# lucidrains/phenaki-pytorch

Hardware: AMD Instinct MI355X
Metric: cvivit_encode_frames_per_sec (higher is better)
Workload: dtype bf16; 1 GPU; BASELINE configs[1]: C-ViViT (dim 512, patch 32, tpatch 2, depth 4+4, LFQ 65536) encode video -> token ids, (8,3,17,256,256) f32 per GPU resident in HBM; global_batch=8, parallelism=batch-shard x1, no data-path collective, hip_graph=True

## Files before the change

phenaki_pytorch_amd/csrc/gemm.hip:

```cpp
#include "gemm_dma.hpp"
#include "gemm_p8.hpp"

namespace pk {

enum { ACT_NONE = 0, ACT_GEGLU = 1, ACT_LEAKY = 2 };

struct GemmEpilogue {
    const float* bias;
    const float* res;
    void* C;
    int ldr, ldc;
    int out_f32;
    int act;
    int vec_ok;
    void* C2;
    int ldc2;
    const float* ln_s; const float* ln_t; float ln_eps;
    const int* row_off; const int* col_off;
    float* stats_out; const float* ln_stats; int stats_np;
    int dup_rows;
};

constexpr int STATS_CHUNK = 32;

// ... 151 lines not shown
    gemm_epilogue<T, TM, TN>(acc, p.M, p.N, e, m0, n0);
}

template <typename Tile>
constexpr int lds_waves_per_simd() {
    const int wgs = 163840 / Tile::SMEM, w = wgs * (Tile::THREADS / 64) / 4;
    return w < 1 ? 1 : (w > 8 ? 8 : w);
}

template <typename T, int TM, int TN, int WM, int WN, int STAGES, int ROWB, int PW, int LNF = 0>
__global__ __launch_bounds__(64 * (WM * WN + PW))
__attribute__((amdgpu_waves_per_eu(lds_waves_per_simd<GemmDma<T, TM, TN, WM, WN, STAGES, ROWB, PW>>(), 8)))
void gemm_dma_kernel(const GemmOperands p, const GemmEpilogue e, int a_nrows) {
    using Tile = GemmDma<T, TM, TN, WM, WN, STAGES, ROWB, PW>;
    extern __shared__ __attribute__((aligned(16))) char smem[];
    const int MT = (p.M + Tile::BM - 1) / Tile::BM, cmax = (MT + 7) / 8, NTn = (p.N + Tile::BN - 1) / Tile::BN;
    const int xcd = blockIdx.x & 7, idx = blockIdx.x >> 3;
    const int mstart = xcd * MT / 8, mcount = (xcd + 1) * MT / 8 - mstart;
    int m0, n0;
    if (p.plain_map) {
        if ((int)blockIdx.x >= MT * NTn) return;
        m0 = (blockIdx.x % MT) * Tile::BM;
        n0 = (blockIdx.x / MT) * Tile::BN;
    } else {
        int ml, ntile;
        if (!xcd_panel_tile(idx, cmax, mcount, NTn, p.panel, ml, ntile)) return;
        m0 = (mstart + ml) * Tile::BM;
        n0 = ntile * Tile::BN;
    }
    PK_TL_KERNEL(0);
    f32x4 acc[TM][TN];
#pragma unroll
    for (int i = 0; i < TM; ++i)
#pragma unroll
        for (int j = 0; j < TN; ++j) acc[i][j] = f32x4{0, 0, 0, 0};
    if constexpr (LNF == 1) {
        float rsum[TM], rsq[TM];
        if (!Tile::template run_stats<2>(p, a_nrows, m0, n0, smem, acc, rsum, rsq)) return;
        gemm_epilogue<T, TM, TN, WN, true>(acc, p.M, p.N, e, m0, n0, rsum, rsq, p.K);
    } else if constexpr (LNF == 2) {
        constexpr int TPR = Tile::THREADS / Tile::BM;
        static_assert(Tile::THREADS == TPR * Tile::BM && (TPR == 2 || TPR == 4), "2 or 4 threads per tile row");
        constexpr int NPRE = 16 / TPR;
        const int srow = threadIdx.x / TPR, sq4 = threadIdx.x % TPR;
        const int per = (e.stats_np + TPR - 1) / TPR, c0 = sq4 * per, c1 = min(c0 + per, e.stats_np);
        const float2* st = reinterpret_cast<const float2*>(e.ln_stats) + (size_t)min(m0 + srow, p.M - 1) * e.stats_np;
        float su = 0.f, sq = 0.f;
        for (int c = c0 + NPRE; c < c1; ++c) { const float2 pr = st[c]; su += pr.x; sq += pr.y; }
        float2 pre[NPRE];
#pragma unroll
        for (int u = 0; u < NPRE; ++u) pre[u] = c0 + u < c1 ? st[c0 + u] : float2{0.f, 0.f};
        if (!Tile::run(p, a_nrows, m0, n0, smem, acc)) return;
#pragma unroll
        for (int u = 0; u < NPRE; ++u) { su += pre[u].x; sq += pre[u].y; }
        su += __shfl_xor(su, 1); sq += __shfl_xor(sq, 1);
        if (TPR == 4) { su += __shfl_xor(su, 2); sq += __shfl_xor(sq, 2); }
        __syncthreads();
        float2* ls = reinterpret_cast<float2*>(smem);
        if (sq4 == 0) ls[srow] = float2{su, sq};
        __syncthreads();
        float rsum[TM], rsq[TM];
        const int lane = threadIdx.x & 63, wm = (threadIdx.x >> 6) / WN;
#pragma unroll
        for (int i = 0; i < TM; ++i) { const float2 pr = ls[wm * 16 * TM + i * 16 + (lane & 15)]; rsum[i] = pr.x; rsq[i] = pr.y; }
        gemm_epilogue<T, TM, TN, WN, true>(acc, p.M, p.N, e, m0, n0, rsum, rsq, p.K);
    } else {
        if (!Tile::run(p, a_nrows, m0, n0, smem, acc)) return;
        PK_TL_KERNEL(1);
        gemm_epilogue<T, TM, TN, WN>(acc, p.M, p.N, e, m0, n0);
        asm volatile("s_waitcnt vmcnt(0)" ::: "memory");
        PK_TL_KERNEL(2);
    }
}

template <typename T, int TM, int TN, int WM, int WN, int STAGES>
__global__ __launch_bounds__(64 * WM * WN)
__attribute__((amdgpu_waves_per_eu(lds_waves_per_simd<GemmDma<T, TM, TN, WM, WN, STAGES, 128, 0>>(), 8)))
void gemm_dma_splitk_kernel(GemmOperands p, GemmEpilogue e, int a_nrows, long batch_a, long batch_w, long batch_c) {
    using Tile = GemmDma<T, TM, TN, WM, WN, STAGES, 128, 0>;
    extern __shared__ __attribute__((aligned(16))) char smem[];
    const int z = blockIdx.y;
    p.A = reinterpret_cast<const char*>(p.A) + (size_t)z * batch_a;
    p.W = reinterpret_cast<const char*>(p.W) + (size_t)z * batch_w;
    e.C = reinterpret_cast<char*>(e.C) + (size_t)z * batch_c;
    if (z != 0) e.bias = nullptr;
    const int MT = (p.M + Tile::BM - 1) / Tile::BM, NTn = (p.N + Tile::BN - 1) / Tile::BN;
// ... 26 lines not shown
    PK_CHECK_LAUNCH();
    return PK_OK;
}

template <typename T, int TM, int TN, int STAGES, int WM = 2, int WN = 2, int ROWB = 128, int PW = 0, int LNF = 0>
static int launch_dma(const GemmOperands& p, const GemmEpilogue& e, int a_nrows, hipStream_t s) {
    using Tile = GemmDma<T, TM, TN, WM, WN, STAGES, ROWB, PW>;
    if (Tile::SMEM > 65536) {
        static LdsOptIn lds;
        if (lds.raise(reinterpret_cast<const void*>(&gemm_dma_kernel<T, TM, TN, WM, WN, STAGES, ROWB, PW, LNF>), Tile::SMEM) != PK_OK) return PK_ELAUNCH;
    }
    const int MT = (p.M + Tile::BM - 1) / Tile::BM, NT = (p.N + Tile::BN - 1) / Tile::BN;
    dim3 grid(8 * ((MT + 7) / 8) * NT);
    GemmOperands pp = p;
    static const int panel_env = [] { const char* e_ = getenv("PK_GEMM_PANEL"); return e_ ? atoi(e_) : -1; }();
    pp.panel = panel_env >= 0 ? panel_env : xcd_panel_rows(Tile::BM, p.K, (int)sizeof(T));
    hipLaunchKernelGGL((gemm_dma_kernel<T, TM, TN, WM, WN, STAGES, ROWB, PW, LNF>), grid, dim3(Tile::THREADS), Tile::SMEM, s, pp, e, a_nrows);
    PK_CHECK_LAUNCH();
    return PK_OK;
}

__global__ __launch_bounds__(512) __attribute__((amdgpu_waves_per_eu(2, 2)))
void gemm_p8_kernel(const GemmOperands p, const GemmEpilogue e, int a_nrows) {
    using Tile = GemmP8;
    extern __shared__ __attribute__((aligned(16))) char smem[];
    const int MT = (p.M + Tile::BM - 1) / Tile::BM, cmax = (MT + 7) / 8, NTn = (p.N + Tile::BN - 1) / Tile::BN;
    const int xcd = blockIdx.x & 7, idx = blockIdx.x >> 3;
    const int mstart = xcd * MT / 8, mcount = (xcd + 1) * MT / 8 - mstart;
    int m0, n0;
    if (p.plain_map) {
        if ((int)blockIdx.x >= MT * NTn) return;
        m0 = (blockIdx.x % MT) * Tile::BM;
        n0 = (blockIdx.x / MT) * Tile::BN;
    } else {
        int ml, ntile;
        if (!xcd_panel_tile(idx, cmax, mcount, NTn, p.panel, ml, ntile)) return;
        m0 = (mstart + ml) * Tile::BM;
        n0 = ntile * Tile::BN;
    }
    Tile::Acc acc;
#pragma unroll
    for (int a = 0; a < 2; ++a)
#pragma unroll
        for (int b = 0; b < 2; ++b)
#pragma unroll
            for (int i = 0; i < 4; ++i)
#pragma unroll
                for (int j = 0; j < 2; ++j) acc[a][b][i][j] = f32x4{0, 0, 0, 0};
    Tile::run(p, a_nrows, m0, n0, smem, acc);
    gemm_epilogue<bf16, 4, 2, 4>(acc[0][0], p.M, p.N, e, m0, n0);
    gemm_epilogue<bf16, 4, 2, 4>(acc[0][1], p.M, p.N, e, m0, n0 + 128);
    gemm_epilogue<bf16, 4, 2, 4>(acc[1][0], p.M, p.N, e, m0 + 128, n0);
    gemm_epilogue<bf16, 4, 2, 4>(acc[1][1], p.M, p.N, e, m0 + 128, n0 + 128);
}

static int launch_p8(const GemmOperands& p, const GemmEpilogue& e, int a_nrows, hipStream_t s) {
    using Tile = GemmP8;
    static LdsOptIn lds;
    if (lds.raise(reinterpret_cast<const void*>(&gemm_p8_kernel), Tile::SMEM) != PK_OK) return PK_ELAUNCH;
    const int MT = (p.M + Tile::BM - 1) / Tile::BM, NT = (p.N + Tile::BN - 1) / Tile::BN;
    dim3 grid(8 * ((MT + 7) / 8) * NT);
    GemmOperands pp = p;
    static const int panel_env = [] { const char* e_ = getenv("PK_GEMM_PANEL"); return e_ ? atoi(e_) : -1; }();
    pp.panel = panel_env >= 0 ? panel_env : xcd_panel_rows(Tile::BM, p.K, (int)sizeof(bf16));
    hipLaunchKernelGGL(gemm_p8_kernel, grid, dim3(Tile::THREADS), Tile::SMEM, s, pp, e, a_nrows);
    PK_CHECK_LAUNCH();
    return PK_OK;
}

__global__ __launch_bounds__(512) __attribute__((amdgpu_waves_per_eu(2, 2)))
void gemm_p8_splitk_kernel(GemmOperands p, GemmEpilogue e, int a_nrows, long batch_a, long batch_w, long batch_c) {
    using Tile = GemmP8;
    extern __shared__ __attribute__((aligned(16))) char smem[];
    const int z = blockIdx.y;
    p.A = reinterpret_cast<const char*>(p.A) + (size_t)z * batch_a;
    p.W = reinterpret_cast<const char*>(p.W) + (size_t)z * batch_w;
    e.C = reinterpret_cast<char*>(e.C) + (size_t)z * batch_c;
    if (z != 0) e.bias = nullptr;
    const int MT = (p.M + Tile::BM - 1) / Tile::BM, NTn = (p.N + Tile::BN - 1) / Tile::BN;
// ... 80 lines not shown
    e.vec_ok = v ? 1 : 0;
    if (C2 && (!v || !out_is_f32 || act == ACT_GEGLU || dtype != 1 || (ldc2 & 3) || (reinterpret_cast<uintptr_t>(C2) & 7))) return PK_EINVAL;
    if ((ln_s == nullptr) != (ln_t == nullptr)) return PK_EINVAL;
    if ((row_off == nullptr) != (col_off == nullptr)) return PK_EINVAL;
    if (row_off && (!v || !out_is_f32 || act == ACT_GEGLU || res || C2)) return PK_EINVAL;
    if (ln_stats && (!ln_s || stats_out || (reinterpret_cast<uintptr_t>(ln_stats) & 7))) return PK_EINVAL;
    if (stats_out && (!v || act == ACT_GEGLU || row_off || (reinterpret_cast<uintptr_t>(stats_out) & 7))) return PK_EINVAL;
    if (dup_rows < 0 || (dup_rows && (!v || act == ACT_GEGLU || row_off || stats_out || dup_rows < M))) return PK_EINVAL;
    hipStream_t s = reinterpret_cast<hipStream_t>(stream);

    const bool dma_ok = dma_possible(dtype, a_is_f32, N, K, lda, ldw, a_nrows);
    if (variant >= 100) { p.plain_map = 1; variant -= 100; }
    if (variant == 0) variant = auto_variant(dtype, a_is_f32, M, N, K, lda, ldw, a_nrows);
    if (variant >= 3 && !dma_ok) return PK_EINVAL;
    if (ln_s) {
        if (!dma_ok || !v || !al16(ln_s) || !al16(ln_t) || a_rows) return PK_EINVAL;
        const bool big = variant == 24 || variant == 2 || variant == 9 || variant == 50;
        if (ln_stats) {
            if (dtype == 1) return big ? launch_dma<bf16, 4, 2, 2, 2, 4, 128, 0, 2>(p, e, a_nrows, s) : launch_dma<bf16, 2, 2, 2, 2, 2, 128, 0, 2>(p, e, a_nrows, s);
            if (dtype == 2) return big ? launch_dma<bf16x3, 4, 4, 2, 2, 2, 128, 0, 2>(p, e, a_nrows, s) : launch_dma<bf16x3, 2, 2, 2, 2, 2, 128, 0, 2>(p, e, a_nrows, s);
            return big ? launch_dma<float, 4, 2, 2, 2, 4, 128, 0, 2>(p, e, a_nrows, s) : launch_dma<float, 2, 2, 2, 2, 2, 128, 0, 2>(p, e, a_nrows, s);
        }
        if (dtype == 1) return big ? launch_dma<bf16, 4, 2, 2, 2, 4, 128, 0, 1>(p, e, a_nrows, s) : launch_dma<bf16, 2, 2, 2, 2, 2, 128, 0, 1>(p, e, a_nrows, s);
        if (dtype == 2) return big ? launch_dma<bf16x3, 4, 4, 2, 2, 2, 128, 0, 1>(p, e, a_nrows, s) : launch_dma<bf16x3, 2, 2, 2, 2, 2, 128, 0, 1>(p, e, a_nrows, s);
        return big ? launch_dma<float, 4, 2, 2, 2, 4, 128, 0, 1>(p, e, a_nrows, s) : launch_dma<float, 2, 2, 2, 2, 2, 128, 0, 1>(p, e, a_nrows, s);
    }
    if (stats_out && !(dma_ok && (variant == 8 || variant == 24 || variant == 27 || variant == 33 || variant == 50 || (variant == 3 && dtype != 1)))) return PK_EINVAL;
    if (dtype == 1) {
        switch (variant) {
            case 1: return a_is_f32 ? launch_v1<bf16, float, 2, 2>(p, e, s) : launch_v1<bf16, bf16, 2, 2>(p, e, s);
            case 2: return a_is_f32 ? launch_v1<bf16, float, 4, 4>(p, e, s) : launch_v1<bf16, bf16, 4, 4>(p, e, s);
// ... 78 lines not shown
```

phenaki_pytorch_amd/csrc/gemm_core.hpp:

```cpp
#pragma once
#include <cstdlib>
#include "common.hpp"

namespace pk {

static inline int krot_default() {
    static const int v = getenv("PK_GEMM_KROT") ? atoi(getenv("PK_GEMM_KROT")) : 1;
    return v;
}

struct GemmOperands {
    const void* A;
    const void* W;
    const int* a_rows;
    int lda, ldw;
    int M, N, K;
    int plain_map;
    int krot;
    int w_gap_from, w_gap_rows;
    int panel;
};

__device__ __forceinline__ bool xcd_panel_tile(int idx, int cmax, int mcount, int NT, int panel, int& ml, int& ntile) {
    if (panel <= 0 || panel >= cmax) { ml = idx % cmax; ntile = idx / cmax; }
    else {
        const int full = cmax / panel;
        int pi = idx / (panel * NT);
        if (pi > full) pi = full;
        const int base = pi * panel;
        const int pl = pi < full ? panel : cmax - base;
        const int r = idx - pi * panel * NT;
        ml = base + r % pl;
        ntile = r / pl;
    }
    return ml < mcount;
}
static inline int xcd_panel_rows(int BM, int K, int esz) {
    const long tile_bytes = (long)BM * K * esz;
    long pnl = (1 << 20) / (tile_bytes > 0 ? tile_bytes : 1);
    return (int)(pnl < 4 ? 4 : pnl);
}

template <typename T, typename TA> struct RawSlot;
template <typename T> struct RawSlot<T, T> { u32x4 v; };
template <> struct RawSlot<bf16, float> { f32x4 a, b; };

template <typename T>
__device__ __forceinline__ void raw_load(RawSlot<T, T>& r, const T* p, bool ok) {
    r.v = ok ? *reinterpret_cast<const u32x4*>(p) : u32x4{0, 0, 0, 0};
// ... 124 lines not shown
```

phenaki_pytorch_amd/csrc/gemm_dma.hpp:

```cpp
#pragma once
#include "gemm_core.hpp"

namespace pk {

__device__ __forceinline__ void dot2acc_bf16(float& d, uint32_t a, uint32_t b) {
    asm("v_dot2c_f32_bf16 %0, %1, %2" : "+v"(d) : "v"(a), "v"(b));
}
__device__ __forceinline__ void frag_stats(const Frag<bf16>& f, float& s, float& q, bool want_sq) {
    const uint32_t w0 = f.v[0], w1 = f.v[1], w2 = f.v[2], w3 = f.v[3];
    const uint32_t ones = 0x3f803f80u;
    dot2acc_bf16(s, w0, ones); dot2acc_bf16(s, w1, ones); dot2acc_bf16(s, w2, ones); dot2acc_bf16(s, w3, ones);
    if (want_sq) { dot2acc_bf16(q, w0, w0); dot2acc_bf16(q, w1, w1); dot2acc_bf16(q, w2, w2); dot2acc_bf16(q, w3, w3); }
}
__device__ __forceinline__ void frag_stats(const Frag<float>& f, float& s, float& q, bool want_sq) {
#pragma unroll
    for (int e = 0; e < 4; ++e) {
        s += f.lo[e] + f.hi[e];
        if (want_sq) q = fmaf(f.lo[e], f.lo[e], fmaf(f.hi[e], f.hi[e], q));
    }
}

#ifdef PK_TIMELINE
__device__ unsigned long long pk_tl[8 * 5 * 40];
#define PK_TL(slot) do { if (tl_on && kt < 38) pk_tl[(tl_wg * 40 + kt) * 5 + (slot)] = __builtin_amdgcn_s_memtime(); } while (0)
// ... 40 lines not shown

    template <int TILES> static __device__ __forceinline__ void wait_tiles() { wait_vmcnt<TILES * IPW>(); }

    static __device__ __forceinline__ void wait_outstanding(int tiles) {
        switch (tiles) {
            case 0: wait_tiles<0>(); break;
            case 1: wait_tiles<1>(); break;
            case 2: wait_tiles<(STAGES > 3 ? 2 : 0)>(); break;
            case 3: wait_tiles<(STAGES > 4 ? 3 : 0)>(); break;
            case 4: wait_tiles<(STAGES > 5 ? 4 : 0)>(); break;
            case 5: wait_tiles<(STAGES > 6 ? 5 : 0)>(); break;
            default: wait_tiles<(STAGES > 7 ? 6 : 0)>(); break;
        }
    }

    static __device__ __forceinline__ bool run(const GemmOperands& p, int a_nrows, int m0, int n0, char* smem, f32x4 (&acc)[TM][TN]) {
        float dummy[TM];
        return run_stats<0>(p, a_nrows, m0, n0, smem, acc, dummy, dummy);
    }

    template <int STATS>
    static __device__ __forceinline__ bool run_stats(const GemmOperands& p, int a_nrows, int m0, int n0, char* smem, f32x4 (&acc)[TM][TN],
                                                     float (&rsum)[TM], float (&rsq)[TM]) {
        const int tid = threadIdx.x, lane = tid & 63;
        const int wave_all = __builtin_amdgcn_readfirstlane(tid >> 6);
        const bool loads = PW == 0 || wave_all >= NW;
        const bool computes = PW == 0 || wave_all < NW;
        const int wave = PW == 0 ? wave_all : (loads ? wave_all - NW : 0);
        const int cw = computes ? wave_all : 0;
        const int wm = cw / WN, wn = cw % WN, g = lane >> 4, lr = lane & 15;
        constexpr int SZ = (int)sizeof(T);

        const uint32_t bytesA = (uint32_t)a_nrows * (uint32_t)p.lda * SZ;
        const uint32_t bytesW = (uint32_t)p.N * (uint32_t)p.ldw * SZ;
        __amdgpu_buffer_rsrc_t rsA = __builtin_amdgcn_make_buffer_rsrc(const_cast<void*>(p.A), 0, bytesA, 0x00020000);
        __amdgpu_buffer_rsrc_t rsW = __builtin_amdgcn_make_buffer_rsrc(const_cast<void*>(p.W), 0, bytesW, 0x00020000);

        const int lrow = lane / SLOTS, lslot = lane % SLOTS;
        const int srcslot = lslot ^ (lrow & 7);
        uint32_t offA[IA], offW[IW];
#pragma unroll
        for (int i = 0; i < IA; ++i) {
            const int row = (wave * IA + i) * RPI + lrow;
            int gm = m0 + row;
            const bool ok = gm < p.M;
            if (ok && p.a_rows) gm = p.a_rows[gm];
            offA[i] = ok ? (uint32_t)gm * (uint32_t)p.lda * SZ + srcslot * 16 : bytesA;
        }
#pragma unroll
        for (int i = 0; i < IW; ++i) {
            const int row = (wave * IW + i) * RPI + lrow;
            const int gn = n0 + row + ((p.w_gap_from > 0 && row >= p.w_gap_from) ? p.w_gap_rows : 0);
            offW[i] = gn < p.N ? (uint32_t)gn * (uint32_t)p.ldw * SZ + srcslot * 16 : bytesW;
        }

        const int nt = (p.K + BK - 1) / BK;
        const int rot = (p.krot && nt > 1) ? (int)(((blockIdx.x >> 3) + blockIdx.y) % (unsigned)nt) : 0;
        const int ktail_bytes = (p.K * SZ) % ROWB;
        const bool slot_in_tail = ktail_bytes == 0 || srcslot * 16 < ktail_bytes;
        auto issue = [&](int kt, int slot) {
            char* base = smem + slot * STAGE_BYTES;
            int kk = kt + rot;
            if (kk >= nt) kk -= nt;
            const int koff = kk * ROWB;
            const bool cut = kk == nt - 1 && !slot_in_tail;
#pragma unroll
            for (int i = 0; i < IA; ++i)
                __builtin_amdgcn_raw_ptr_buffer_load_lds(rsA, (lds_ptr)(base + (wave * IA + i) * 1024), 16, cut ? bytesA : offA[i], koff, 0, 0);
#pragma unroll
            for (int i = 0; i < IW; ++i)
                __builtin_amdgcn_raw_ptr_buffer_load_lds(rsW, (lds_ptr)(base + BM * ROWB + (wave * IW + i) * 1024), 16, offW[i], koff, 0, 0);
        };

        if (STATS) {
#pragma unroll
            for (int i = 0; i < TM; ++i) { rsum[i] = 0.f; rsq[i] = 0.f; }
        }
        const int pre = nt < STAGES - 1 ? nt : STAGES - 1;
        if (loads)
            for (int s = 0; s < pre; ++s) issue(s, s);
        if (PW > 0 && computes) __builtin_amdgcn_s_setprio(1);
#ifdef PK_TIMELINE
        const int tl_wg = pk_tl_wg();
        const bool tl_on = tl_wg >= 0 && tid == 0;
#endif
        for (int kt = 0; kt < nt; ++kt) {
            const int issued = (kt + STAGES - 1 < nt) ? kt + STAGES - 1 : nt;
            PK_TL(0);
            if (loads) wait_outstanding(issued - (kt + 1));
            PK_TL(1);
            __builtin_amdgcn_s_barrier();
            PK_TL(2);
            if (loads && kt + STAGES - 1 < nt) issue(kt + STAGES - 1, (kt + STAGES - 1) % STAGES);
            PK_TL(3);
            if (!computes) continue;
            const char* a = smem + (kt % STAGES) * STAGE_BYTES;
            const char* w = a + BM * ROWB;
#pragma unroll
            for (int c = 0; c < CH; ++c) {
                Frag<T> fa[TM], fw[TN];
#pragma unroll
                for (int i = 0; i < TM; ++i) lds_frag_a<T>(fa[i], a, wm * 16 * TM + i * 16 + lr, c, g);
#pragma unroll
                for (int j = 0; j < TN; ++j) lds_frag_w<T>(fw[j], w, wn * 16 * TN + j * 16 + lr, c, g);
#pragma unroll
                for (int i = 0; i < TM; ++i)
#pragma unroll
                    for (int j = 0; j < TN; ++j) acc[i][j] = mma(fw[j], fa[i], acc[i][j]);
// ... 7 lines not shown
        if (STATS) {
#pragma unroll
            for (int i = 0; i < TM; ++i) {
                rsum[i] += __shfl_xor(rsum[i], 16, 64);
                rsum[i] += __shfl_xor(rsum[i], 32, 64);
                if (STATS > 1) {
                    rsq[i] += __shfl_xor(rsq[i], 16, 64);
                    rsq[i] += __shfl_xor(rsq[i], 32, 64);
                }
            }
        }
        asm volatile("s_waitcnt lgkmcnt(0)" ::: "memory");
        __builtin_amdgcn_s_barrier();
        return computes;
    }
};

}
```

phenaki_pytorch_amd/csrc/qkv.hip:

```cpp
#include "gemm_dma.hpp"

namespace pk {

struct QkvArgs {
    const void* xq; const void* xkv;
    const void* wq; const void* wkv;
    int ld, ldw;
    int M, K, h, nseq;
    const float* q_scale; const float* k_scale; float scale;
    void* Qp; void* Kp; void* Vt;
    int nq_pad, nk_pad;
    int krot;
    const float* q_ln_s;
};

template <typename T, int TM> using QkvTileT = GemmDma<T, TM, 4, 4, 1, 2, 128>;

template <typename T, int TM>
__global__ __launch_bounds__(256) void qkv_project_kernel(const QkvArgs a) {
    using QkvTile = QkvTileT<T, TM>;
    typedef typename ImageOf<T>::type TI;
    constexpr int BM = 64 * TM;
    extern __shared__ __attribute__((aligned(16))) char smem[];
    const int MT = (a.M + BM - 1) / BM, cmax = (MT + 7) / 8;
// ... 2 lines not shown
    const int ml = idx % cmax;
    if (ml >= mcount) return;
    const int m0 = (mstart + ml) * BM;
    const int nt = idx / cmax;
    const bool is_q = nt < a.h;
    const int kind = is_q ? 0 : (nt < 2 * a.h ? 1 : 2);
    const int hh = nt - kind * a.h;
    GemmOperands p;
    p.A = is_q ? a.xq : a.xkv;
    p.W = is_q ? a.wq : a.wkv;
    p.a_rows = nullptr;
    p.lda = a.ld; p.ldw = a.ldw;
    p.M = a.M; p.N = is_q ? a.h * 64 : 2 * a.h * 64; p.K = a.K;
    p.plain_map = 0;
    p.krot = a.krot;
    p.w_gap_from = 0; p.w_gap_rows = 0; p.panel = 0;
    const int n0 = is_q ? hh * 64 : (kind == 1 ? hh * 64 : (a.h + hh) * 64);

    f32x4 acc[TM][4];
#pragma unroll
    for (int i = 0; i < TM; ++i)
#pragma unroll
        for (int j = 0; j < 4; ++j) acc[i][j] = f32x4{0, 0, 0, 0};
    const int lane = threadIdx.x & 63, wave = threadIdx.x >> 6, g = lane >> 4, lr = lane & 15;
    if (is_q && a.q_ln_s) {
        float rsum[TM], rsq[TM];
        (void)QkvTile::template run_stats<1>(p, a.M, m0, n0, smem, acc, rsum, rsq);
        f32x4 s4[4];
#pragma unroll
        for (int j = 0; j < 4; ++j) s4[j] = *reinterpret_cast<const f32x4*>(a.q_ln_s + n0 + j * 16 + g * 4);
#pragma unroll
        for (int i = 0; i < TM; ++i) {
            const float mean = rsum[i] / (float)a.K;
#pragma unroll
            for (int j = 0; j < 4; ++j)
#pragma unroll
                for (int r = 0; r < 4; ++r) acc[i][j][r] -= mean * s4[j][r];
        }
    } else {
        (void)QkvTile::run(p, a.M, m0, n0, smem, acc);
    }

// ... 85 lines not shown
```

phenaki_pytorch_amd/csrc/qkv_attn.hip:

```cpp
#include "gemm_dma.hpp"

namespace pk {

struct QkvAttnArgs {
    const void* xq; const void* xkv;
    const void* wq; const void* wkv;
    int ld, ldw;
    int S, n, h, K;
    int spt;
    const float* q_scale; const float* k_scale; float scale;
    const float* bias; long bias_hstride; int bias_ld;
    const float* slopes; int causal;
    void* O; int ldo;
    uint32_t recip;
    const float* q_ln_s;
};

template <typename T> using QaTile = GemmDma<T, 1, 4, 4, 1, 2, 128>;
template <typename T> using QaKvTile = GemmDma<T, 1, 8, 4, 1, 2, 128>;
constexpr int QA_SMEM = QaKvTile<bf16>::SMEM;
static_assert(QaKvTile<bf16x3>::SMEM == QA_SMEM, "the split-bf16 ring has the same bytes");

constexpr int QA_PLANE = 8192;
template <typename T> struct QaImg { static constexpr int PLANES = 1; };
template <> struct QaImg<bf16x3> { static constexpr int PLANES = 2; };
__device__ __forceinline__ void qa_put4(bf16, char* img, int off, f32x4 v) {
    *reinterpret_cast<u32x2*>(img + off) = u32x2{pack_bf2(v[0], v[1]), pack_bf2(v[2], v[3])};
}
__device__ __forceinline__ void qa_put4(bf16x3, char* img, int off, f32x4 v) {
    const uint32_t h0 = pack_bf2(v[0], v[1]), h1 = pack_bf2(v[2], v[3]);
// ... 8 lines not shown
    *reinterpret_cast<u16*>(img + off) = h;
    *reinterpret_cast<u16*>(img + QA_PLANE + off) = f2bf(v - bf2f(h));
}
__device__ __forceinline__ void qa_get(Frag<bf16>& f, const char* img, int off) { f.v = *reinterpret_cast<const u32x4*>(img + off); }
__device__ __forceinline__ void qa_get(Frag<bf16x3>& f, const char* img, int off) {
    f.hi = *reinterpret_cast<const u32x4*>(img + off);
    f.lo = *reinterpret_cast<const u32x4*>(img + QA_PLANE + off);
}

__device__ __forceinline__ int qa_kperm(int f, int i) { return (f >> 1) * 32 + (i >> 2) * 8 + (f & 1) * 4 + (i & 3); }
__device__ __forceinline__ int qa_ksw(int row) { return ((row >> 1) & 1) | (((row >> 3) & 3) << 1); }

template <typename T>
__device__ __forceinline__ void qa_project_q(const GemmOperands& p, int M, int m0, int hh, int K, const float* q_scale, float scale,
                                             const float* q_ln_s, char* smem, char* Qs) {
    const int lane = threadIdx.x & 63, g = lane >> 4, lr = lane & 15;
    const int rq = __builtin_amdgcn_readfirstlane(threadIdx.x >> 6) * 16 + lr;
    f32x4 acc[1][4];
#pragma unroll
    for (int j = 0; j < 4; ++j) acc[0][j] = f32x4{0, 0, 0, 0};
    if (q_ln_s) {
        float rsum[1], rsq[1];
        (void)QaTile<T>::template run_stats<1>(p, M, m0, hh * 64, smem, acc, rsum, rsq);
        const float mean = rsum[0] / (float)K;
#pragma unroll
        for (int j = 0; j < 4; ++j) {
            const f32x4 s4 = *reinterpret_cast<const f32x4*>(q_ln_s + hh * 64 + j * 16 + g * 4);
#pragma unroll
            for (int r = 0; r < 4; ++r) acc[0][j][r] -= mean * s4[r];
        }
    } else {
        (void)QaTile<T>::run(p, M, m0, hh * 64, smem, acc);
    }
    float ss = 0.f;
#pragma unroll
    for (int j = 0; j < 4; ++j)
#pragma unroll
        for (int r = 0; r < 4; ++r) ss += acc[0][j][r] * acc[0][j][r];
    ss += __shfl_xor(ss, 16, 64);
    ss += __shfl_xor(ss, 32, 64);
    const float inv = scale / fmaxf(sqrtf(ss), 1e-12f);
#pragma unroll
    for (int j = 0; j < 4; ++j) {
        const f32x4 sc = *reinterpret_cast<const f32x4*>(q_scale + j * 16 + g * 4);
        f32x4 v = acc[0][j];
#pragma unroll
        for (int r = 0; r < 4; ++r) v[r] *= inv * sc[r];
        const int slot = (2 * j + (g >> 1)) ^ (rq & 7);
        qa_put4(T{}, Qs, rq * 128 + (slot << 4) + (g & 1) * 8, v);
    }
}

template <typename T>
__global__ __launch_bounds__(256) void qkv_attn_kernel(const QkvAttnArgs a) {
    extern __shared__ __attribute__((aligned(16))) char smem[];
    constexpr int NPL = QaImg<T>::PLANES;
    char* Qs = smem;
    char* Ks = smem;
    char* Vts = smem + NPL * QA_PLANE;
    const int R = a.spt * a.n;
    const int tiles = (a.S + a.spt - 1) / a.spt;
    const int xcd = blockIdx.x & 7, idx = blockIdx.x >> 3;
    const int tile = (idx / a.h) * 8 + xcd, hh = idx % a.h;
    if (tile >= tiles) return;
    const int M = a.S * a.n;
    const int m0 = tile * R;
    const int lane = threadIdx.x & 63, g = lane >> 4, lr = lane & 15;
    const int wave = __builtin_amdgcn_readfirstlane(threadIdx.x >> 6);
    const int rq = wave * 16 + lr;

    GemmOperands p;
    p.a_rows = nullptr;
    p.lda = a.ld; p.ldw = a.ldw;
    p.M = M; p.K = a.K;
    p.plain_map = 0; p.krot = 0;
    p.w_gap_from = 0; p.w_gap_rows = 0;

    p.A = a.xq; p.W = a.wq; p.N = a.h * 64;
// ... 115 lines not shown
    }
    if (!qvalid) return;
    const float inv = 1.0f / ls;
    T* orow = reinterpret_cast<T*>(a.O) + (size_t)(m0 + rq) * a.ldo + hh * 64;
#pragma unroll
    for (int df = 0; df < 4; ++df) store4(orow + df * 16 + g * 4, o[df] * inv);
}

struct QAttnCachedArgs {
    const void* xq; const void* wq; int ld, ldw;
    int S, n, h, K;
    const float* q_scale; float scale; const float* q_ln_s;
    const void* Kp; const void* Vt; int nk_pad, nk, nnull;
    const unsigned char* kmask; int n_kv;
    void* O; int ldo;
};

template <typename T, bool NK64>
__global__ __launch_bounds__(256) void q_attn_cached_kernel(const QAttnCachedArgs a) {
    extern __shared__ __attribute__((aligned(16))) char smem[];
    constexpr int NPL = QaImg<T>::PLANES;
    char* Qs = smem + QaTile<T>::SMEM;
    char* Ks = Qs + NPL * QA_PLANE;
    char* Vts = smem;
    const int M = a.S * a.n;
    const int tiles = M / 64;
    const int xcd = blockIdx.x & 7, idx = blockIdx.x >> 3;
    const int tile = (idx / a.h) * 8 + xcd, hh = idx % a.h;
    if (tile >= tiles) return;
    const int m0 = tile * 64;
    const int s = m0 / a.n;
    const int lane = threadIdx.x & 63, g = lane >> 4, lr = lane & 15;
    const int wave = __builtin_amdgcn_readfirstlane(threadIdx.x >> 6);
    const int rq = wave * 16 + lr;

    GemmOperands p;
    p.a_rows = nullptr;
    p.lda = a.ld; p.ldw = a.ldw;
    p.M = M; p.K = a.K;
    p.plain_map = 0; p.krot = 0;
    p.w_gap_from = 0; p.w_gap_rows = 0;
    p.A = a.xq; p.W = a.wq; p.N = a.h * 64;
    qa_project_q<T>(p, M, m0, hh, a.K, a.q_scale, a.scale, a.q_ln_s, smem, Qs);

    {
        const size_t sh = (size_t)s * a.h + hh;
        const int row = threadIdx.x >> 2, part = threadIdx.x & 3;
        const u32x4 zero = u32x4{0, 0, 0, 0};
        if constexpr (NPL == 1) {
            const bf16* krow = reinterpret_cast<const bf16*>(a.Kp) + (sh * a.nk_pad + row) * 64;
            const bf16* vrow = reinterpret_cast<const bf16*>(a.Vt) + (sh * 64 + row) * a.nk_pad;
#pragma unroll
            for (int q = 0; q < 2; ++q) {
                const int slot = part * 2 + q;
                const u32x4 kv = row < a.nk_pad ? *reinterpret_cast<const u32x4*>(krow + slot * 8) : zero;
                *reinterpret_cast<u32x4*>(Ks + row * 128 + ((slot ^ qa_ksw(row)) << 4)) = kv;
                const u32x4 vv = slot * 8 < a.nk_pad ? *reinterpret_cast<const u32x4*>(vrow + slot * 8) : zero;
                *reinterpret_cast<u32x4*>(Vts + row * 128 + ((slot ^ (row & 7)) << 4)) = vv;
// ... 95 lines not shown
        (reinterpret_cast<uintptr_t>(O) & (dtype == 1 ? 7 : 15)) || (bias && mis(bias))) return PK_EALIGN;
    if (ldw < (K + bk - 1) / bk * bk) return PK_EINVAL;
    const long M = (long)S * n;
    if ((size_t)M * ld * esz >= 0xFFFFFFF0ull || (size_t)2 * h * 64 * ldw * esz >= 0xFFFFFFF0ull) return PK_EINVAL;
    QkvAttnArgs a;
    a.xq = xq; a.xkv = xkv; a.wq = wq; a.wkv = wkv; a.ld = ld; a.ldw = ldw;
    a.S = S; a.n = n; a.h = h; a.K = K; a.spt = 64 / n;
    a.q_scale = q_scale; a.k_scale = k_scale; a.scale = scale;
    a.bias = bias; a.bias_hstride = bias_hstride; a.bias_ld = bias_ld;
    a.slopes = slopes; a.causal = causal;
    a.O = O; a.ldo = ldo;
    a.recip = (65536u + (uint32_t)n - 1u) / (uint32_t)n;
    a.q_ln_s = q_ln_s;
    if (q_ln_s && mis(q_ln_s)) return PK_EALIGN;
    const int tiles = (S + a.spt - 1) / a.spt;
    dim3 grid(8 * ((tiles + 7) / 8) * h);
    hipStream_t st = reinterpret_cast<hipStream_t>(stream);
    if (dtype == 1) hipLaunchKernelGGL(qkv_attn_kernel<bf16>, grid, dim3(256), QA_SMEM, st, a);
    else hipLaunchKernelGGL(qkv_attn_kernel<bf16x3>, grid, dim3(256), QA_SMEM, st, a);
    PK_CHECK_LAUNCH();
    return PK_OK;
}

extern "C" int pk_q_attn_cached(int dtype, const void* xq, int ld, const void* wq, int ldw, int S, int n, int h, int K, const float* q_scale,
                                float scale, const float* q_ln_s, const void* Kp, const void* Vt, int nk_pad, int n_kv, int nnull,
                                const unsigned char* kmask, void* O, int ldo, void* stream) {
    if (dtype != 1 && dtype != 2) return PK_EINVAL;
    if (!xq || !wq || !q_scale || !Kp || !Vt || !O || S <= 0 || n <= 0 || (n & 63) || h <= 0 || K <= 0 || n_kv <= 0 || nnull < 0) return PK_EINVAL;
    const int nk = nnull + n_kv;
    if (nk > 64 || nk_pad < nk || nk_pad > 64 || (nk_pad & 31)) return PK_EINVAL;
    auto mis = [](const void* ptr) { return (reinterpret_cast<uintptr_t>(ptr) & 15) != 0; };
    const int q = dtype == 1 ? 7 : 3, bk = dtype == 1 ? 64 : 32, esz = dtype == 1 ? 2 : 4;
    if ((K & q) || (ld & q) || (ldw & q) || (ldo & 3) || mis(xq) || mis(wq) || mis(q_scale) || mis(Kp) || mis(Vt) ||
        (reinterpret_cast<uintptr_t>(O) & (dtype == 1 ? 7 : 15)) || (q_ln_s && mis(q_ln_s))) return PK_EALIGN;
    if (dtype == 2 && ((reinterpret_cast<uintptr_t>(Kp) | reinterpret_cast<uintptr_t>(Vt)) & 127)) return PK_EALIGN;
    if (ldw < (K + bk - 1) / bk * bk) return PK_EINVAL;
    const long M = (long)S * n;
    if ((size_t)M * ld * esz >= 0xFFFFFFF0ull || (size_t)h * 64 * ldw * esz >= 0xFFFFFFF0ull) return PK_EINVAL;
    QAttnCachedArgs a{xq, wq, ld, ldw, S, n, h, K, q_scale, scale, q_ln_s, Kp, Vt, nk_pad, nk, nnull, kmask, n_kv, O, ldo};
    const int tiles = (int)(M / 64);
    dim3 grid(8 * ((tiles + 7) / 8) * h);
    hipStream_t st = reinterpret_cast<hipStream_t>(stream);
    if (dtype == 1) {
        constexpr int lds = QaTile<bf16>::SMEM + 2 * QA_PLANE;
        if (nk_pad > 32) hipLaunchKernelGGL((q_attn_cached_kernel<bf16, true>), grid, dim3(256), lds, st, a);
        else hipLaunchKernelGGL((q_attn_cached_kernel<bf16, false>), grid, dim3(256), lds, st, a);
    } else {
        constexpr int lds = QaTile<bf16x3>::SMEM + 4 * QA_PLANE;
        if (nk_pad > 32) hipLaunchKernelGGL((q_attn_cached_kernel<bf16x3, true>), grid, dim3(256), lds, st, a);
        else hipLaunchKernelGGL((q_attn_cached_kernel<bf16x3, false>), grid, dim3(256), lds, st, a);
    }
    PK_CHECK_LAUNCH();
    return PK_OK;
}
// ... 1 lines not shown
```

Before: 170,600 frames/s.

## Split DMA GEMM into begin/loop to issue prologue loads before tile setup

Refactors the DMA GEMM tile into a Ring state with a begin step that issues the prologue buffer-to-LDS loads early, and a loop step that consumes them. Prefetches of LN statistics and Q projection are reordered so global loads overlap. Tile index mapping replaces integer divisions with host-precomputed magic reciprocals, and a trailing vmcnt wait is compiled only under timeline builds. It also batches a_rows gather loads and relaxes the LN-with-a_rows restriction, which adds a functional path and some correctness risk.

```diff
diff --git a/phenaki_pytorch_amd/csrc/gemm.hip b/phenaki_pytorch_amd/csrc/gemm.hip
--- a/phenaki_pytorch_amd/csrc/gemm.hip
+++ b/phenaki_pytorch_amd/csrc/gemm.hip
@@ -189,21 +189,21 @@
 void gemm_dma_kernel(const GemmOperands p, const GemmEpilogue e, int a_nrows) {
     using Tile = GemmDma<T, TM, TN, WM, WN, STAGES, ROWB, PW>;
     extern __shared__ __attribute__((aligned(16))) char smem[];
-    const int MT = (p.M + Tile::BM - 1) / Tile::BM, cmax = (MT + 7) / 8, NTn = (p.N + Tile::BN - 1) / Tile::BN;
-    const int xcd = blockIdx.x & 7, idx = blockIdx.x >> 3;
-    const int mstart = xcd * MT / 8, mcount = (xcd + 1) * MT / 8 - mstart;
+    PK_TL_KERNEL(0);
+    gemm_operands_resident(p, a_nrows);
     int m0, n0;
     if (p.plain_map) {
-        if ((int)blockIdx.x >= MT * NTn) return;
-        m0 = (blockIdx.x % MT) * Tile::BM;
-        n0 = (blockIdx.x / MT) * Tile::BN;
+        if ((int)blockIdx.x >= p.map.MT * p.map.NT) return;
+        m0 = (blockIdx.x % p.map.MT) * Tile::BM;
+        n0 = (blockIdx.x / p.map.MT) * Tile::BN;
     } else {
-        int ml, ntile;
-        if (!xcd_panel_tile(idx, cmax, mcount, NTn, p.panel, ml, ntile)) return;
-        m0 = (mstart + ml) * Tile::BM;
+        int mtile, ntile;
+        if (!xcd_panel_tile(p.map, blockIdx.x, mtile, ntile)) return;
+        m0 = mtile * Tile::BM;
         n0 = ntile * Tile::BN;
     }
-    PK_TL_KERNEL(0);
+    typename Tile::Ring ring;
+    Tile::begin(p, a_nrows, m0, n0, smem, ring);
     f32x4 acc[TM][TN];
 #pragma unroll
     for (int i = 0; i < TM; ++i)
@@ -211,7 +211,7 @@
         for (int j = 0; j < TN; ++j) acc[i][j] = f32x4{0, 0, 0, 0};
     if constexpr (LNF == 1) {
         float rsum[TM], rsq[TM];
-        if (!Tile::template run_stats<2>(p, a_nrows, m0, n0, smem, acc, rsum, rsq)) return;
+        if (!Tile::template loop_stats<2>(ring, acc, rsum, rsq)) return;
         gemm_epilogue<T, TM, TN, WN, true>(acc, p.M, p.N, e, m0, n0, rsum, rsq, p.K);
     } else if constexpr (LNF == 2) {
         constexpr int TPR = Tile::THREADS / Tile::BM;
@@ -220,12 +220,12 @@
         const int srow = threadIdx.x / TPR, sq4 = threadIdx.x % TPR;
         const int per = (e.stats_np + TPR - 1) / TPR, c0 = sq4 * per, c1 = min(c0 + per, e.stats_np);
         const float2* st = reinterpret_cast<const float2*>(e.ln_stats) + (size_t)min(m0 + srow, p.M - 1) * e.stats_np;
+        float2 pre[NPRE];
+#pragma unroll
+        for (int u = 0; u < NPRE; ++u) pre[u] = c0 + u < c1 ? st[c0 + u] : float2{0.f, 0.f};
+        if (!Tile::loop(ring, acc)) return;
         float su = 0.f, sq = 0.f;
         for (int c = c0 + NPRE; c < c1; ++c) { const float2 pr = st[c]; su += pr.x; sq += pr.y; }
-        float2 pre[NPRE];
-#pragma unroll
-        for (int u = 0; u < NPRE; ++u) pre[u] = c0 + u < c1 ? st[c0 + u] : float2{0.f, 0.f};
-        if (!Tile::run(p, a_nrows, m0, n0, smem, acc)) return;
 #pragma unroll
         for (int u = 0; u < NPRE; ++u) { su += pre[u].x; sq += pre[u].y; }
         su += __shfl_xor(su, 1); sq += __shfl_xor(sq, 1);
@@ -240,11 +240,13 @@
         for (int i = 0; i < TM; ++i) { const float2 pr = ls[wm * 16 * TM + i * 16 + (lane & 15)]; rsum[i] = pr.x; rsq[i] = pr.y; }
         gemm_epilogue<T, TM, TN, WN, true>(acc, p.M, p.N, e, m0, n0, rsum, rsq, p.K);
     } else {
-        if (!Tile::run(p, a_nrows, m0, n0, smem, acc)) return;
+        if (!Tile::loop(ring, acc)) return;
         PK_TL_KERNEL(1);
         gemm_epilogue<T, TM, TN, WN>(acc, p.M, p.N, e, m0, n0);
+#ifdef PK_TIMELINE
         asm volatile("s_waitcnt vmcnt(0)" ::: "memory");
         PK_TL_KERNEL(2);
+#endif
     }
 }
 
@@ -301,7 +303,7 @@
     dim3 grid(8 * ((MT + 7) / 8) * NT);
     GemmOperands pp = p;
     static const int panel_env = [] { const char* e_ = getenv("PK_GEMM_PANEL"); return e_ ? atoi(e_) : -1; }();
-    pp.panel = panel_env >= 0 ? panel_env : xcd_panel_rows(Tile::BM, p.K, (int)sizeof(T));
+    pp.map = xcd_map_make(p.M, p.N, Tile::BM, Tile::BN, panel_env >= 0 ? panel_env : xcd_panel_rows(Tile::BM, p.K, (int)sizeof(T)));
     hipLaunchKernelGGL((gemm_dma_kernel<T, TM, TN, WM, WN, STAGES, ROWB, PW, LNF>), grid, dim3(Tile::THREADS), Tile::SMEM, s, pp, e, a_nrows);
     PK_CHECK_LAUNCH();
     return PK_OK;
@@ -311,18 +313,15 @@
 void gemm_p8_kernel(const GemmOperands p, const GemmEpilogue e, int a_nrows) {
     using Tile = GemmP8;
     extern __shared__ __attribute__((aligned(16))) char smem[];
-    const int MT = (p.M + Tile::BM - 1) / Tile::BM, cmax = (MT + 7) / 8, NTn = (p.N + Tile::BN - 1) / Tile::BN;
-    const int xcd = blockIdx.x & 7, idx = blockIdx.x >> 3;
-    const int mstart = xcd * MT / 8, mcount = (xcd + 1) * MT / 8 - mstart;
     int m0, n0;
     if (p.plain_map) {
-        if ((int)blockIdx.x >= MT * NTn) return;
-        m0 = (blockIdx.x % MT) * Tile::BM;
-        n0 = (blockIdx.x / MT) * Tile::BN;
+        if ((int)blockIdx.x >= p.map.MT * p.map.NT) return;
+        m0 = (blockIdx.x % p.map.MT) * Tile::BM;
+        n0 = (blockIdx.x / p.map.MT) * Tile::BN;
     } else {
-        int ml, ntile;
-        if (!xcd_panel_tile(idx, cmax, mcount, NTn, p.panel, ml, ntile)) return;
-        m0 = (mstart + ml) * Tile::BM;
+        int mtile, ntile;
+        if (!xcd_panel_tile(p.map, blockIdx.x, mtile, ntile)) return;
+        m0 = mtile * Tile::BM;
         n0 = ntile * Tile::BN;
     }
     Tile::Acc acc;
@@ -349,7 +348,7 @@
     dim3 grid(8 * ((MT + 7) / 8) * NT);
     GemmOperands pp = p;
     static const int panel_env = [] { const char* e_ = getenv("PK_GEMM_PANEL"); return e_ ? atoi(e_) : -1; }();
-    pp.panel = panel_env >= 0 ? panel_env : xcd_panel_rows(Tile::BM, p.K, (int)sizeof(bf16));
+    pp.map = xcd_map_make(p.M, p.N, Tile::BM, Tile::BN, panel_env >= 0 ? panel_env : xcd_panel_rows(Tile::BM, p.K, (int)sizeof(bf16)));
     hipLaunchKernelGGL(gemm_p8_kernel, grid, dim3(Tile::THREADS), Tile::SMEM, s, pp, e, a_nrows);
     PK_CHECK_LAUNCH();
     return PK_OK;
@@ -460,7 +459,7 @@
     if (variant == 0) variant = auto_variant(dtype, a_is_f32, M, N, K, lda, ldw, a_nrows);
     if (variant >= 3 && !dma_ok) return PK_EINVAL;
     if (ln_s) {
-        if (!dma_ok || !v || !al16(ln_s) || !al16(ln_t) || a_rows) return PK_EINVAL;
+        if (!dma_ok || !v || !al16(ln_s) || !al16(ln_t)) return PK_EINVAL;
         const bool big = variant == 24 || variant == 2 || variant == 9 || variant == 50;
         if (ln_stats) {
             if (dtype == 1) return big ? launch_dma<bf16, 4, 2, 2, 2, 4, 128, 0, 2>(p, e, a_nrows, s) : launch_dma<bf16, 2, 2, 2, 2, 2, 128, 0, 2>(p, e, a_nrows, s);
diff --git a/phenaki_pytorch_amd/csrc/gemm_core.hpp b/phenaki_pytorch_amd/csrc/gemm_core.hpp
--- a/phenaki_pytorch_amd/csrc/gemm_core.hpp
+++ b/phenaki_pytorch_amd/csrc/gemm_core.hpp
@@ -8,6 +8,14 @@
     static const int v = getenv("PK_GEMM_KROT") ? atoi(getenv("PK_GEMM_KROT")) : 1;
     return v;
 }
+
+struct XcdMap {
+    int MT, NT;
+    int cmax;
+    int panel;
+    int full, tail;
+    uint32_t r_pnt, r_panel, r_tail;
+};
 
 struct GemmOperands {
     const void* A;
@@ -18,21 +26,49 @@
     int plain_map;
     int krot;
     int w_gap_from, w_gap_rows;
-    int panel;
+    XcdMap map;
 };
 
-__device__ __forceinline__ bool xcd_panel_tile(int idx, int cmax, int mcount, int NT, int panel, int& ml, int& ntile) {
-    if (panel <= 0 || panel >= cmax) { ml = idx % cmax; ntile = idx / cmax; }
-    else {
-        const int full = cmax / panel;
-        int pi = idx / (panel * NT);
-        if (pi > full) pi = full;
-        const int base = pi * panel;
-        const int pl = pi < full ? panel : cmax - base;
-        const int r = idx - pi * panel * NT;
-        ml = base + r % pl;
-        ntile = r / pl;
-    }
+__device__ __forceinline__ void gemm_operands_resident(const GemmOperands& p, int a_nrows) {
+    asm volatile("" ::"s"(p.A), "s"(p.W), "s"(p.a_rows), "s"(p.lda), "s"(p.ldw), "s"(p.M), "s"(p.N), "s"(p.K), "s"(p.plain_map), "s"(p.krot),
+                 "s"(p.w_gap_from), "s"(p.w_gap_rows), "s"(a_nrows));
+    asm volatile("" ::"s"(p.map.MT), "s"(p.map.NT), "s"(p.map.panel), "s"(p.map.full), "s"(p.map.tail), "s"(p.map.r_pnt), "s"(p.map.r_panel),
+                 "s"(p.map.r_tail));
+}
+
+static inline uint32_t magic_recip(uint32_t d) { return d <= 1 ? 0xFFFFFFFFu : (uint32_t)(0x100000000ull / d); }
+__device__ __forceinline__ uint32_t magic_div(uint32_t n, uint32_t d, uint32_t r, uint32_t& rem) {
+    uint32_t q = __umulhi(n, r);
+    rem = n - q * d;
+    if (rem >= d) { ++q; rem -= d; }
+    return q;
+}
+
+static inline XcdMap xcd_map_make(int M, int N, int BM, int BN, int panel) {
+    XcdMap m;
+    m.MT = (M + BM - 1) / BM; m.NT = (N + BN - 1) / BN;
+    m.cmax = (m.MT + 7) / 8;
+    m.panel = (panel <= 0 || panel >= m.cmax) ? m.cmax : panel;
+    m.full = m.cmax / m.panel;
+    m.tail = m.cmax - m.full * m.panel;
+    m.r_pnt = magic_recip((uint32_t)m.panel * (uint32_t)m.NT);
+    m.r_panel = magic_recip((uint32_t)m.panel);
+    m.r_tail = magic_recip((uint32_t)m.tail);
+    return m;
+}
+__device__ __forceinline__ bool xcd_panel_tile(const XcdMap& m, uint32_t block, int& mtile, int& ntile) {
+    const uint32_t xcd = block & 7u, idx = block >> 3;
+    const uint32_t mstart = (xcd * (uint32_t)m.MT) >> 3, mcount = (((xcd + 1) * (uint32_t)m.MT) >> 3) - mstart;
+    const uint32_t pnt = (uint32_t)m.panel * (uint32_t)m.NT;
+    uint32_t r;
+    uint32_t pi = magic_div(idx, pnt, m.r_pnt, r);
+    if (pi > (uint32_t)m.full) { pi = m.full; r = idx - pi * pnt; }
+    const bool whole = pi < (uint32_t)m.full;
+    const uint32_t pl = whole ? (uint32_t)m.panel : (uint32_t)m.tail;
+    uint32_t rm;
+    ntile = (int)magic_div(r, pl, whole ? m.r_panel : m.r_tail, rm);
+    const uint32_t ml = pi * (uint32_t)m.panel + rm;
+    mtile = (int)(mstart + ml);
     return ml < mcount;
 }
 static inline int xcd_panel_rows(int BM, int K, int esz) {
diff --git a/phenaki_pytorch_amd/csrc/gemm_dma.hpp b/phenaki_pytorch_amd/csrc/gemm_dma.hpp
--- a/phenaki_pytorch_amd/csrc/gemm_dma.hpp
+++ b/phenaki_pytorch_amd/csrc/gemm_dma.hpp
@@ -78,71 +78,97 @@
         }
     }
 
-    static __device__ __forceinline__ bool run(const GemmOperands& p, int a_nrows, int m0, int n0, char* smem, f32x4 (&acc)[TM][TN]) {
-        float dummy[TM];
-        return run_stats<0>(p, a_nrows, m0, n0, smem, acc, dummy, dummy);
-    }
-
-    template <int STATS>
-    static __device__ __forceinline__ bool run_stats(const GemmOperands& p, int a_nrows, int m0, int n0, char* smem, f32x4 (&acc)[TM][TN],
-                                                     float (&rsum)[TM], float (&rsq)[TM]) {
+    struct Ring {
+        const void* A; const void* W;
+        uint32_t bytesA, bytesW;
+        uint32_t offA[IA], offW[IW];
+        char* smem;
+        int nt, rot, pre;
+        int wave, cw;
+        bool loads, computes, slot_in_tail;
+    };
+
+    static __device__ __forceinline__ void issue(const Ring& r, int kt, int slot) {
+        const __amdgpu_buffer_rsrc_t rsA = __builtin_amdgcn_make_buffer_rsrc(const_cast<void*>(r.A), 0, r.bytesA, 0x00020000);
+        const __amdgpu_buffer_rsrc_t rsW = __builtin_amdgcn_make_buffer_rsrc(const_cast<void*>(r.W), 0, r.bytesW, 0x00020000);
+        char* base = r.smem + slot * STAGE_BYTES;
+        int kk = kt + r.rot;
+        if (kk >= r.nt) kk -= r.nt;
+        const int koff = kk * ROWB;
+        const bool cut = kk == r.nt - 1 && !r.slot_in_tail;
+#pragma unroll
+        for (int i = 0; i < IA; ++i)
+            __builtin_amdgcn_raw_ptr_buffer_load_lds(rsA, (lds_ptr)(base + (r.wave * IA + i) * 1024), 16, cut ? r.bytesA : r.offA[i], koff, 0, 0);
+#pragma unroll
+        for (int i = 0; i < IW; ++i)
+            __builtin_amdgcn_raw_ptr_buffer_load_lds(rsW, (lds_ptr)(base + BM * ROWB + (r.wave * IW + i) * 1024), 16, r.offW[i], koff, 0, 0);
+    }
+
+    static __device__ __forceinline__ void begin(const GemmOperands& p, int a_nrows, int m0, int n0, char* smem, Ring& r) {
         const int tid = threadIdx.x, lane = tid & 63;
         const int wave_all = __builtin_amdgcn_readfirstlane(tid >> 6);
-        const bool loads = PW == 0 || wave_all >= NW;
-        const bool computes = PW == 0 || wave_all < NW;
-        const int wave = PW == 0 ? wave_all : (loads ? wave_all - NW : 0);
-        const int cw = computes ? wave_all : 0;
-        const int wm = cw / WN, wn = cw % WN, g = lane >> 4, lr = lane & 15;
+        r.loads = PW == 0 || wave_all >= NW;
+        r.computes = PW == 0 || wave_all < NW;
+        r.wave = PW == 0 ? wave_all : (r.loads ? wave_all - NW : 0);
+        r.cw = r.computes ? wave_all : 0;
+        r.smem = smem;
         constexpr int SZ = (int)sizeof(T);
+        const int wave = r.wave;
 
         const uint32_t bytesA = (uint32_t)a_nrows * (uint32_t)p.lda * SZ;
         const uint32_t bytesW = (uint32_t)p.N * (uint32_t)p.ldw * SZ;
-        __amdgpu_buffer_rsrc_t rsA = __builtin_amdgcn_make_buffer_rsrc(const_cast<void*>(p.A), 0, bytesA, 0x00020000);
-        __amdgpu_buffer_rsrc_t rsW = __builtin_amdgcn_make_buffer_rsrc(const_cast<void*>(p.W), 0, bytesW, 0x00020000);
+        r.A = p.A; r.W = p.W; r.bytesA = bytesA; r.bytesW = bytesW;
 
         const int lrow = lane / SLOTS, lslot = lane % SLOTS;
         const int srcslot = lslot ^ (lrow & 7);
-        uint32_t offA[IA], offW[IW];
-#pragma unroll
-        for (int i = 0; i < IA; ++i) {
-            const int row = (wave * IA + i) * RPI + lrow;
-            int gm = m0 + row;
-            const bool ok = gm < p.M;
-            if (ok && p.a_rows) gm = p.a_rows[gm];
-            offA[i] = ok ? (uint32_t)gm * (uint32_t)p.lda * SZ + srcslot * 16 : bytesA;
+        if (p.a_rows) {
+            int gm[IA];
+#pragma unroll
+            for (int i = 0; i < IA; ++i) gm[i] = p.a_rows[min(m0 + (wave * IA + i) * RPI + lrow, p.M - 1)];
+#pragma unroll
+            for (int i = 0; i < IA; ++i) {
+                const bool ok = m0 + (wave * IA + i) * RPI + lrow < p.M;
+                r.offA[i] = ok ? (uint32_t)gm[i] * (uint32_t)p.lda * SZ + srcslot * 16 : bytesA;
+            }
+        } else {
+#pragma unroll
+            for (int i = 0; i < IA; ++i) {
+                const int gm = m0 + (wave * IA + i) * RPI + lrow;
+                r.offA[i] = gm < p.M ? (uint32_t)gm * (uint32_t)p.lda * SZ + srcslot * 16 : bytesA;
+            }
         }
 #pragma unroll
         for (int i = 0; i < IW; ++i) {
             const int row = (wave * IW + i) * RPI + lrow;
             const int gn = n0 + row + ((p.w_gap_from > 0 && row >= p.w_gap_from) ? p.w_gap_rows : 0);
-            offW[i] = gn < p.N ? (uint32_t)gn * (uint32_t)p.ldw * SZ + srcslot * 16 : bytesW;
-        }
-
-        const int nt = (p.K + BK - 1) / BK;
-        const int rot = (p.krot && nt > 1) ? (int)(((blockIdx.x >> 3) + blockIdx.y) % (unsigned)nt) : 0;
+            r.offW[i] = gn < p.N ? (uint32_t)gn * (uint32_t)p.ldw * SZ + srcslot * 16 : bytesW;
+        }
+
+        r.nt = (p.K + BK - 1) / BK;
+        r.rot = 0;
+        if (p.krot && r.nt > 1) r.rot = (int)(((blockIdx.x >> 3) + blockIdx.y) % (unsigned)r.nt);
         const int ktail_bytes = (p.K * SZ) % ROWB;
-        const bool slot_in_tail = ktail_bytes == 0 || srcslot * 16 < ktail_bytes;
-        auto issue = [&](int kt, int slot) {
-            char* base = smem + slot * STAGE_BYTES;
-            int kk = kt + rot;
-            if (kk >= nt) kk -= nt;
-            const int koff = kk * ROWB;
-            const bool cut = kk == nt - 1 && !slot_in_tail;
-#pragma unroll
-            for (int i = 0; i < IA; ++i)
-                __builtin_amdgcn_raw_ptr_buffer_load_lds(rsA, (lds_ptr)(base + (wave * IA + i) * 1024), 16, cut ? bytesA : offA[i], koff, 0, 0);
-#pragma unroll
-            for (int i = 0; i < IW; ++i)
-                __builtin_amdgcn_raw_ptr_buffer_load_lds(rsW, (lds_ptr)(base + BM * ROWB + (wave * IW + i) * 1024), 16, offW[i], koff, 0, 0);
-        };
-
+        r.slot_in_tail = ktail_bytes == 0 || srcslot * 16 < ktail_bytes;
+        r.pre = r.nt < STAGES - 1 ? r.nt : STAGES - 1;
+        if (r.loads)
+            for (int s = 0; s < r.pre; ++s) issue(r, s, s);
+    }
+
+    static __device__ __forceinline__ bool loop(const Ring& r, f32x4 (&acc)[TM][TN]) {
+        float dummy[TM];
+        return loop_stats<0>(r, acc, dummy, dummy);
+    }
+    template <int STATS>
+    static __device__ __forceinline__ bool loop_stats(const Ring& r, f32x4 (&acc)[TM][TN], float (&rsum)[TM], float (&rsq)[TM]) {
+        const int tid = threadIdx.x, lane = tid & 63;
+        const bool loads = r.loads, computes = r.computes;
+        const int wm = r.cw / WN, wn = r.cw % WN, g = lane >> 4, lr = lane & 15;
+        const int nt = r.nt;
+        char* smem = r.smem;
         if (STATS) {
 #pragma unroll
             for (int i = 0; i < TM; ++i) { rsum[i] = 0.f; rsq[i] = 0.f; }
         }
-        const int pre = nt < STAGES - 1 ? nt : STAGES - 1;
-        if (loads)
-            for (int s = 0; s < pre; ++s) issue(s, s);
         if (PW > 0 && computes) __builtin_amdgcn_s_setprio(1);
 #ifdef PK_TIMELINE
         const int tl_wg = pk_tl_wg();
@@ -155,7 +181,7 @@
             PK_TL(1);
             __builtin_amdgcn_s_barrier();
             PK_TL(2);
-            if (loads && kt + STAGES - 1 < nt) issue(kt + STAGES - 1, (kt + STAGES - 1) % STAGES);
+            if (loads && kt + STAGES - 1 < nt) issue(r, kt + STAGES - 1, (kt + STAGES - 1) % STAGES);
             PK_TL(3);
             if (!computes) continue;
             const char* a = smem + (kt % STAGES) * STAGE_BYTES;
@@ -193,6 +219,12 @@
         __builtin_amdgcn_s_barrier();
         return computes;
     }
+
+    static __device__ __forceinline__ bool run(const GemmOperands& p, int a_nrows, int m0, int n0, char* smem, f32x4 (&acc)[TM][TN]) {
+        Ring r;
+        begin(p, a_nrows, m0, n0, smem, r);
+        return loop(r, acc);
+    }
 };
 
 }
diff --git a/phenaki_pytorch_amd/csrc/qkv.hip b/phenaki_pytorch_amd/csrc/qkv.hip
--- a/phenaki_pytorch_amd/csrc/qkv.hip
+++ b/phenaki_pytorch_amd/csrc/qkv.hip
@@ -40,7 +40,7 @@
     p.M = a.M; p.N = is_q ? a.h * 64 : 2 * a.h * 64; p.K = a.K;
     p.plain_map = 0;
     p.krot = a.krot;
-    p.w_gap_from = 0; p.w_gap_rows = 0; p.panel = 0;
+    p.w_gap_from = 0; p.w_gap_rows = 0;
     const int n0 = is_q ? hh * 64 : (kind == 1 ? hh * 64 : (a.h + hh) * 64);
 
     f32x4 acc[TM][4];
@@ -51,7 +51,9 @@
     const int lane = threadIdx.x & 63, wave = threadIdx.x >> 6, g = lane >> 4, lr = lane & 15;
     if (is_q && a.q_ln_s) {
         float rsum[TM], rsq[TM];
-        (void)QkvTile::template run_stats<1>(p, a.M, m0, n0, smem, acc, rsum, rsq);
+        typename QkvTile::Ring ring;
+        QkvTile::begin(p, a.M, m0, n0, smem, ring);
+        (void)QkvTile::template loop_stats<1>(ring, acc, rsum, rsq);
         f32x4 s4[4];
 #pragma unroll
         for (int j = 0; j < 4; ++j) s4[j] = *reinterpret_cast<const f32x4*>(a.q_ln_s + n0 + j * 16 + g * 4);
diff --git a/phenaki_pytorch_amd/csrc/qkv_attn.hip b/phenaki_pytorch_amd/csrc/qkv_attn.hip
--- a/phenaki_pytorch_amd/csrc/qkv_attn.hip
+++ b/phenaki_pytorch_amd/csrc/qkv_attn.hip
@@ -14,6 +14,7 @@
     void* O; int ldo;
     uint32_t recip;
     const float* q_ln_s;
+    int tiles; uint32_t r_h;
 };
 
 template <typename T> using QaTile = GemmDma<T, 1, 4, 4, 1, 2, 128>;
@@ -52,6 +53,8 @@
 template <typename T>
 __device__ __forceinline__ void qa_project_q(const GemmOperands& p, int M, int m0, int hh, int K, const float* q_scale, float scale,
                                              const float* q_ln_s, char* smem, char* Qs) {
+    typename QaTile<T>::Ring ring;
+    QaTile<T>::begin(p, M, m0, hh * 64, smem, ring);
     const int lane = threadIdx.x & 63, g = lane >> 4, lr = lane & 15;
     const int rq = __builtin_amdgcn_readfirstlane(threadIdx.x >> 6) * 16 + lr;
     f32x4 acc[1][4];
@@ -59,7 +62,7 @@
     for (int j = 0; j < 4; ++j) acc[0][j] = f32x4{0, 0, 0, 0};
     if (q_ln_s) {
         float rsum[1], rsq[1];
-        (void)QaTile<T>::template run_stats<1>(p, M, m0, hh * 64, smem, acc, rsum, rsq);
+        (void)QaTile<T>::template loop_stats<1>(ring, acc, rsum, rsq);
         const float mean = rsum[0] / (float)K;
 #pragma unroll
         for (int j = 0; j < 4; ++j) {
@@ -68,7 +71,7 @@
             for (int r = 0; r < 4; ++r) acc[0][j][r] -= mean * s4[r];
         }
     } else {
-        (void)QaTile<T>::run(p, M, m0, hh * 64, smem, acc);
+        (void)QaTile<T>::loop(ring, acc);
     }
     float ss = 0.f;
 #pragma unroll
@@ -97,9 +100,10 @@
     char* Ks = smem;
     char* Vts = smem + NPL * QA_PLANE;
     const int R = a.spt * a.n;
-    const int tiles = (a.S + a.spt - 1) / a.spt;
-    const int xcd = blockIdx.x & 7, idx = blockIdx.x >> 3;
-    const int tile = (idx / a.h) * 8 + xcd, hh = idx % a.h;
+    const int tiles = a.tiles;
+    const int xcd = blockIdx.x & 7;
+    uint32_t hrem;
+    const int tile = (int)magic_div(blockIdx.x >> 3, a.h, a.r_h, hrem) * 8 + xcd, hh = (int)hrem;
     if (tile >= tiles) return;
     const int M = a.S * a.n;
     const int m0 = tile * R;
@@ -245,6 +249,7 @@
     const void* Kp; const void* Vt; int nk_pad, nk, nnull;
     const unsigned char* kmask; int n_kv;
     void* O; int ldo;
+    uint32_t r_h;
 };
 
 template <typename T, bool NK64>
@@ -256,11 +261,11 @@
     char* Vts = smem;
     const int M = a.S * a.n;
     const int tiles = M / 64;
-    const int xcd = blockIdx.x & 7, idx = blockIdx.x >> 3;
-    const int tile = (idx / a.h) * 8 + xcd, hh = idx % a.h;
+    const int xcd = blockIdx.x & 7;
+    uint32_t hrem;
+    const int tile = (int)magic_div(blockIdx.x >> 3, a.h, a.r_h, hrem) * 8 + xcd, hh = (int)hrem;
     if (tile >= tiles) return;
     const int m0 = tile * 64;
-    const int s = m0 / a.n;
     const int lane = threadIdx.x & 63, g = lane >> 4, lr = lane & 15;
     const int wave = __builtin_amdgcn_readfirstlane(threadIdx.x >> 6);
     const int rq = wave * 16 + lr;
@@ -273,6 +278,7 @@
     p.w_gap_from = 0; p.w_gap_rows = 0;
     p.A = a.xq; p.W = a.wq; p.N = a.h * 64;
     qa_project_q<T>(p, M, m0, hh, a.K, a.q_scale, a.scale, a.q_ln_s, smem, Qs);
+    const int s = m0 / a.n;
 
     {
         const size_t sh = (size_t)s * a.h + hh;
@@ -398,6 +404,7 @@
     a.q_ln_s = q_ln_s;
     if (q_ln_s && mis(q_ln_s)) return PK_EALIGN;
     const int tiles = (S + a.spt - 1) / a.spt;
+    a.tiles = tiles; a.r_h = magic_recip((uint32_t)h);
     dim3 grid(8 * ((tiles + 7) / 8) * h);
     hipStream_t st = reinterpret_cast<hipStream_t>(stream);
     if (dtype == 1) hipLaunchKernelGGL(qkv_attn_kernel<bf16>, grid, dim3(256), QA_SMEM, st, a);
@@ -421,7 +428,7 @@
     if (ldw < (K + bk - 1) / bk * bk) return PK_EINVAL;
     const long M = (long)S * n;
     if ((size_t)M * ld * esz >= 0xFFFFFFF0ull || (size_t)h * 64 * ldw * esz >= 0xFFFFFFF0ull) return PK_EINVAL;
-    QAttnCachedArgs a{xq, wq, ld, ldw, S, n, h, K, q_scale, scale, q_ln_s, Kp, Vt, nk_pad, nk, nnull, kmask, n_kv, O, ldo};
+    QAttnCachedArgs a{xq, wq, ld, ldw, S, n, h, K, q_scale, scale, q_ln_s, Kp, Vt, nk_pad, nk, nnull, kmask, n_kv, O, ldo, magic_recip((uint32_t)h)};
     const int tiles = (int)(M / 64);
     dim3 grid(8 * ((tiles + 7) / 8) * h);
     hipStream_t st = reinterpret_cast<hipStream_t>(stream);
```

Result: faster. 175,400 frames/s, median of 5 (+2.8%).
